# yxtay/transformer-recommenders

Hardware: AMD Instinct MI355X
Metric: user-sequences/sec (train step) MovieLens-1M seq200 d128 @1/2/4/8 GPU (higher is better)
Workload: dtype bf16; 1 GPU; MovieLens-1M-shaped: 3883 items, seq_len=200, d_model=128, 4-layer causal BERT (heads=4, ffn=512), InfoNCELoss over in-batch shared negatives, AdamW; per_gpu_batch=512, global_batch=512, seq_len=200, lengths=dense, loss_heads_evaluated=all 7 + LogitsStatistics (reference training_step), parallelism=dp1, launch=eager launches

## Files before the change

### transformer-recommenders_amd/csrc/common.h

```cpp
#pragma once
#include <hip/hip_runtime.h>
#include <stdint.h>

#include "xfmr_hip.h"

typedef __attribute__((ext_vector_type(8))) __bf16 bf16x8;
typedef __attribute__((ext_vector_type(4))) __bf16 bf16x4;
typedef __attribute__((ext_vector_type(2))) __bf16 bf16x2;
typedef __attribute__((ext_vector_type(16))) float f32x16;

#define XF_WAVE 64

#define XF_LAUNCH_CHECK()                                   \
  do {                                                      \
    if (hipGetLastError() != hipSuccess) return XFMR_EHIP;  \
  } while (0)

static inline bool xf_aligned16(const void* p) { return (reinterpret_cast<uintptr_t>(p) & 15u) == 0; }

__device__ __forceinline__ int xf_lane() { return threadIdx.x & 63; }

__device__ __forceinline__ int xf_acc_row(int r, int lane) { return (r & 3) + 8 * (r >> 2) + 4 * (lane >> 5); }

struct PrecBF16 {
// ... 397 lines not shown
  return fmaf(-p, e, 0.5f);
}
__device__ __forceinline__ float xf_gelu(float x) {
  float e;
  const float ax = fabsf(x);
  return fmaf(ax, xf_phi_minus_half(ax, x, e), 0.5f * x);
}
__device__ __forceinline__ float xf_gelu_both(float x, float& grad) {
  float e;
  const float ax = fabsf(x);
  const float h = xf_phi_minus_half(ax, x, e);
  grad = fmaf(x * 0.3989422804014327f, e, 0.5f + copysignf(h, x));
  return fmaf(ax, h, 0.5f * x);
}
__device__ __forceinline__ float xf_gelu_grad(float x) {
  float e;
  const float h = xf_phi_minus_half(fabsf(x), x, e);
  return fmaf(x * 0.3989422804014327f, e, 0.5f + copysignf(h, x));
}
__device__ __forceinline__ float xf_softplus(float x) {
  return fmaxf(x, 0.f) + 0.6931471805599453f * xf_log2(1.f + xf_exp2(-fabsf(x) * 1.4426950408889634f));
}
__device__ __forceinline__ float xf_sigmoid(float x) {
  const float t = xf_exp2(-fabsf(x) * 1.4426950408889634f);
  return xf_rcp(1.f + t) * (x >= 0.f ? 1.f : t);
}

__device__ __forceinline__ void xf_store_tile_T(float* scratch, const f32x16& acc, float mul, float* base, int64_t stride,
                                             int row0, int row_end) {
  const int lane = xf_lane();
#pragma unroll
  for (int r = 0; r < 16; ++r) scratch[(lane & 31) * 33 + xf_acc_row(r, lane)] = acc[r] * mul;
  __builtin_amdgcn_s_waitcnt(0xc07f);
  __builtin_amdgcn_wave_barrier();
  const int j = lane >> 1, half = lane & 1;
  if (row0 + j < row_end) {
    float* dst = base + (int64_t)(row0 + j) * stride + 16 * half;
#pragma unroll
    for (int u = 0; u < 4; ++u) {
      float4 v;
      v.x = scratch[j * 33 + 16 * half + 4 * u + 0];
      v.y = scratch[j * 33 + 16 * half + 4 * u + 1];
      v.z = scratch[j * 33 + 16 * half + 4 * u + 2];
      v.w = scratch[j * 33 + 16 * half + 4 * u + 3];
      *reinterpret_cast<float4*>(dst + 4 * u) = v;
    }
  }
  __builtin_amdgcn_wave_barrier();
}

__device__ __forceinline__ void xf_store_tile_T(float* scratch, const f32x16& acc, float mul, __bf16* base,
                                                int64_t stride, int row0, int row_end) {
  const int lane = xf_lane();
#pragma unroll
  for (int r = 0; r < 16; ++r) scratch[(lane & 31) * 33 + xf_acc_row(r, lane)] = acc[r] * mul;
  __builtin_amdgcn_s_waitcnt(0xc07f);
  __builtin_amdgcn_wave_barrier();
  const int j = lane >> 1, half = lane & 1;
  if (row0 + j < row_end) {
    __bf16* dst = base + (int64_t)(row0 + j) * stride + 16 * half;
#pragma unroll
    for (int u = 0; u < 2; ++u) {
      bf16x8 v;
#pragma unroll
      for (int e = 0; e < 8; ++e) v[e] = (__bf16)scratch[j * 33 + 16 * half + 8 * u + e];
      *reinterpret_cast<bf16x8*>(dst + 8 * u) = v;
    }
  }
  __builtin_amdgcn_wave_barrier();
}
template <bool S16>
__device__ __forceinline__ void xf_store_tile_T_at(float* scratch, const f32x16& acc, float mul, void* base,
                                                   int64_t off, int64_t stride, int row0, int row_end) {
  if (S16) xf_store_tile_T(scratch, acc, mul, reinterpret_cast<__bf16*>(base) + off, stride, row0, row_end);
  else xf_store_tile_T(scratch, acc, mul, reinterpret_cast<float*>(base) + off, stride, row0, row_end);
}


typedef __attribute__((ext_vector_type(4))) short xf_s16x4;

template <int H>
struct SwzImg {
  static constexpr int CPR = H / 8;
  __device__ static __forceinline__ int swz(int r) {
    if (CPR == 4) return (r >> 2) & 3;
    if (CPR >= 16) return ((r & 3) << 2) | ((r >> 2) & 3);
    return (((r >> 1) & 1) << 2) | ((r & 1) << 1) | ((r >> 2) & 1);
  }
  __device__ static __forceinline__ int off(int r, int c) { return r * H + 8 * (c ^ swz(r)); }

  __device__ static __forceinline__ void tile_nreg(f32x16& acc, const __bf16* A, int arow0, const bf16x8* breg) {
    const int l = xf_lane(), r = arow0 + (l & 31), hh = l >> 5;
#pragma unroll
    for (int s = 0; s < H / 16; ++s) {
      const bf16x8 a = *reinterpret_cast<const bf16x8*>(A + off(r, 2 * s + hh));
      acc = __builtin_amdgcn_mfma_f32_32x32x16_bf16(a, breg[s], acc, 0, 0, 0);
    }
  }
  __device__ static __forceinline__ void tile_nt(f32x16& acc, const __bf16* A, int arow0, const __bf16* B, int brow0) {
    const int l = xf_lane(), ra = arow0 + (l & 31), rb = brow0 + (l & 31), hh = l >> 5;
#pragma unroll
    for (int s = 0; s < H / 16; ++s) {
      const bf16x8 a = *reinterpret_cast<const bf16x8*>(A + off(ra, 2 * s + hh));
      const bf16x8 b = *reinterpret_cast<const bf16x8*>(B + off(rb, 2 * s + hh));
      acc = __builtin_amdgcn_mfma_f32_32x32x16_bf16(a, b, acc, 0, 0, 0);
    }
  }
  __device__ static __forceinline__ void tile_xb_tr(f32x16& acc, const __bf16* img, int hsub, int jrow0,
                                                    const f32x16& x) {
    const int l = xf_lane(), g16 = l >> 4, hh = g16 >> 1, li = l & 15, q = li >> 2, p = li & 3;
    const int col = hsub * 32 + 16 * (g16 & 1) + 4 * p;
    const int c = col >> 3, within = col & 7;
#pragma unroll
    for (int s = 0; s < 2; ++s) {
      bf16x8 b;
#pragma unroll
      for (int j = 0; j < 8; ++j) b[j] = (__bf16)x[8 * s + j];
      union { xf_s16x4 v[2]; bf16x8 f; } a;
#pragma unroll
      for (int t = 0; t < 2; ++t) {
        const int row = jrow0 + 16 * s + 8 * t + 4 * hh + q;
        const __bf16* ptr = img + off(row, c) + within;
        a.v[t] = __builtin_amdgcn_ds_read_tr16_b64_v4i16(
            (__attribute__((address_space(3))) xf_s16x4*)(ptr));
      }
      acc = __builtin_amdgcn_mfma_f32_32x32x16_bf16(a.f, b, acc, 0, 0, 0);
    }
  }
  __device__ static __forceinline__ bf16x8 frag_tr(const __bf16* img, int col0, int k0) {
    const int l = xf_lane(), g16 = l >> 4, li = l & 15, q = li >> 2, p = li & 3;
    const int col = col0 + 16 * (g16 & 1) + 4 * p;
    const int c = col >> 3, within = col & 7;
    union { xf_s16x4 v[2]; bf16x8 f; } a;
#pragma unroll
    for (int t = 0; t < 2; ++t) {
      const int row = k0 + 8 * (g16 >> 1) + 4 * t + q;
      a.v[t] = __builtin_amdgcn_ds_read_tr16_b64_v4i16(
          (__attribute__((address_space(3))) xf_s16x4*)(img + off(row, c) + within));
    }
    return a.f;
  }
  __device__ static __forceinline__ int gather_row(int row0) { return row0 + xf_lane() / CPR; }
  __device__ static __forceinline__ int gather_src_chunk(int row) { return (xf_lane() % CPR) ^ swz(row); }
  static constexpr int kRowsPerInstr = 64 / CPR;
};

__device__ __forceinline__ void xf_glds16(const void* gsrc, void* lds_base) {
  __builtin_amdgcn_global_load_lds((const __attribute__((address_space(1))) void*)gsrc,
                                   (__attribute__((address_space(3))) void*)lds_base, 16, 0, 0);
}
__device__ __forceinline__ void xf_glds16_raw_so(const void* sbase, uint32_t voff, void* lds_base) {
  const unsigned dst = (unsigned)(uintptr_t)(__attribute__((address_space(3))) void*)lds_base;
  unsigned keep;
  asm volatile("s_mov_b32 %0, m0\n\ts_mov_b32 m0, %3\n\ts_nop 0\n\tglobal_load_lds_dwordx4 %1, %2\n\ts_mov_b32 m0, %0"
               : "=&s"(keep)
               : "v"(voff), "s"(sbase), "s"(dst)
               : "memory");
}
template <int N>
__device__ __forceinline__ void xf_wait_vm() {
  __builtin_amdgcn_s_waitcnt((N & 0xF) | ((N >> 4) << 14) | (7 << 4) | (0xF << 8));
}
__device__ __forceinline__ void xf_glds16_raw(const void* gsrc, void* lds_base) {
  const unsigned dst = (unsigned)(uintptr_t)(__attribute__((address_space(3))) void*)lds_base;
  unsigned keep;
  asm volatile("s_mov_b32 %0, m0\n\ts_mov_b32 m0, %2\n\ts_nop 0\n\tglobal_load_lds_dwordx4 %1, off\n\ts_mov_b32 m0, %0"
               : "=&s"(keep)
               : "v"(gsrc), "s"(dst)
               : "memory");
}
```

### transformer-recommenders_amd/csrc/gemm.hip

```cpp
#include <stdio.h>
#include <stdlib.h>

#include <algorithm>
#include <type_traits>

#include "internal.h"

#define XF_PIN_SCALAR(x) asm volatile("" : "+v"(x))
#ifndef XF_LN_DIAG
#define XF_LN_DIAG 0
#endif
#ifndef XF_GEMM_PF
#define XF_GEMM_PF 1
#endif
#ifndef XF_DW_PF
#define XF_DW_PF 1
#endif
#ifdef XF_FFN_STAMP
#define XF_STAMP(i) do { if (stamp_on) st_buf[(i)] = __builtin_readcyclecounter(); } while (0)
#else
#define XF_STAMP(i) do {} while (0)
#endif
#ifndef XF_FFN_ASM_BARRIER
#define XF_FFN_ASM_BARRIER 1
// ... 703 lines not shown
            v[q].x += ax.x; v[q].y += ax.y; v[q].z += ax.z; v[q].w += ax.w;
          } else if (EPI == EPI_GELU_GRAD) {
            if (g.aux_grad) {
              v[q].x *= ax.x; v[q].y *= ax.y; v[q].z *= ax.z; v[q].w *= ax.w;
            } else {
              v[q].x *= xf_gelu_grad(ax.x); v[q].y *= xf_gelu_grad(ax.y);
              v[q].z *= xf_gelu_grad(ax.z); v[q].w *= xf_gelu_grad(ax.w);
            }
          }
        }
        if (EPI == EPI_GELU) st_out(g.C2, o, d);
        st_out(g.C, zoff + o, v);
      }
      __builtin_amdgcn_s_waitcnt(0xc07f);
      __builtin_amdgcn_wave_barrier();
    }
  }
}
template <class P, int BM, int BN, int BK, bool TA, bool TB, int EPI, uint32_t S>
__global__ __launch_bounds__(256, (epi_res_ln(EPI) || EPI == EPI_DX_LNBWD) ? XF_LN_EPI_MIN_WAVES : 1) void gemm_kernel(const GemmArgs g_in) {
  gemm_body<P, BM, BN, BK, TA, TB, EPI, S>(g_in, (int)blockIdx.x);
}
struct GemmGroup { GemmArgs g[4]; int start[5]; };
template <class P, int BM, int BN, int BK, bool TA, bool TB, int EPI, uint32_t S>
__global__ __launch_bounds__(256, 1) void gemm_group_kernel(const GemmGroup p) {
  const int b = (int)blockIdx.x;
  const int i = (b >= p.start[1]) + (b >= p.start[2]) + (b >= p.start[3]);
  gemm_body<P, BM, BN, BK, TA, TB, EPI, S>(p.g[i], b - p.start[i]);
}

struct FfnFwdArgs {
  const __bf16* X;
  const __bf16* W1;
  const float* b1;
  const __bf16* W2;
  __bf16* U;
  __bf16* G;
  int I;
  GemmArgs e;
  unsigned long long* stamps;
};

template <int N, class F>
__device__ __forceinline__ void xf_static_for(F&& fn) {
  if constexpr (N > 0) {
    xf_static_for<N - 1>(fn);
    fn(std::integral_constant<int, N - 1>{});
  }
}
template <int CH>
struct WeightChunk {
  static constexpr int NW = CH / 16, PC = CH / 8, H = 128, LDH = H + 8, LDC = CH + 8;
  bf16x8 reg[NW];
  __device__ __forceinline__ void load_w1(const __bf16* W1, int c, int tid) {
    xf_static_for<NW>([&](auto ic) {
      constexpr int i = decltype(ic)::value;
      const int p = tid + i * 256, row = p >> 4, ch = p & 15;
      reg[i] = *reinterpret_cast<const bf16x8*>(W1 + (int64_t)(c * CH + row) * H + ch * 8);
    });
  }
  __device__ __forceinline__ void commit_w1(__bf16* sW, int tid) const {
    xf_static_for<NW>([&](auto ic) {
      constexpr int i = decltype(ic)::value;
      const int p = tid + i * 256, row = p >> 4, ch = p & 15;
      *reinterpret_cast<bf16x8*>(sW + row * LDH + ch * 8) = reg[i];
    });
  }
  __device__ __forceinline__ void load_w2(const __bf16* W2, int I, int c, int tid) {
    xf_static_for<NW>([&](auto ic) {
      constexpr int i = decltype(ic)::value;
      const int p = tid + i * 256, row = p / PC, ch = p % PC;
      reg[i] = *reinterpret_cast<const bf16x8*>(W2 + (int64_t)row * I + c * CH + ch * 8);
    });
  }
  __device__ __forceinline__ void commit_w2(__bf16* sW, int tid) const {
    xf_static_for<NW>([&](auto ic) {
      constexpr int i = decltype(ic)::value;
      const int p = tid + i * 256, row = p / PC, ch = p % PC;
      *reinterpret_cast<bf16x8*>(sW + row * LDC + ch * 8) = reg[i];
    });
  }
};

template <int CH, bool RE = false>
__global__ __launch_bounds__(256, CH == 128 ? XF_FFN_MIN_WAVES : 3) void ffn_fwd_fused_kernel(const FfnFwdArgs f_in) {
  FfnFwdArgs f = f_in;
  XF_CHAIN_PRIO();
  f.e.drop = xf_drop_resolve(f.e.drop);
  constexpr int H = 128, LDH = H + 8, LDC = CH + 8, BM = 64;
  constexpr int NJ = CH / 64;
  constexpr int W_ELEMS = CH * LDH > H * LDC ? CH * LDH : H * LDC;
  __shared__ __attribute__((aligned(16))) __bf16 sG[BM * LDC];
  __shared__ __attribute__((aligned(16))) __bf16 sW[W_ELEMS];
  __shared__ float sB1[1024];
  static_assert(W_ELEMS >= BM * LDH, "the x tile is staged through sW");
  static_assert(W_ELEMS * 2 >= 4 * 16 * 68 * 4 + 128 * 4, "the LayerNorm epilogue's scratch aliases sW");
  using FR = Frag<PrecBF16, false>;
  const int lane = threadIdx.x & 63, wid = threadIdx.x >> 6, tid = threadIdx.x;
  const int wr = wid >> 1, wc = wid & 1;
  const TileIdx tix = tile_of(1, f.e.nt_m, 1);
  if (!tix.valid) return;
  const int64_t m0 = xf_tile_rows(f.e, tix.m, BM);
  const int64_t M = f.e.M;
  const int I = f.I, nchunk = I / CH;
#ifdef XF_FFN_STAMP
  const bool stamp_on = f.stamps && threadIdx.x == 0;
  unsigned long long* st_buf = f.stamps + (int64_t)blockIdx.x * 64;
#endif
  XF_STAMP(0);

  WeightChunk<CH> wa, wb;
  constexpr int PC = CH / 8;

  {
    uint4 xr[4];
#pragma unroll
    for (int i = 0; i < 4; ++i) {
      const int p = tid + i * 256, row = p >> 4, ch = p & 15;
      xr[i] = make_uint4(0u, 0u, 0u, 0u);
      if (m0 + row < M) xr[i] = *reinterpret_cast<const uint4*>(f.X + (m0 + row) * H + ch * 8);
    }
    wa.load_w1(f.W1, 0, tid);
    wb.load_w2(f.W2, I, 0, tid);
    for (int i = tid; i < I; i += 256) sB1[i] = f.b1[i];
#pragma unroll
    for (int i = 0; i < 4; ++i) {
      const int p = tid + i * 256, row = p >> 4, ch = p & 15;
      *reinterpret_cast<uint4*>(sW + row * LDH + ch * 8) = xr[i];
    }
  }
  __syncthreads();
  bf16x8 xa[H / 16];
#pragma unroll
  for (int ks = 0; ks < H / 16; ++ks) xa[ks] = FR::get(sW, LDH, wr * 32, ks * 16);
  XF_STAMP(1);

  f32x16 accy[2];
#pragma unroll
  for (int j = 0; j < 2; ++j)
#pragma unroll
    for (int r = 0; r < 16; ++r) accy[j][r] = 0.f;

  for (int c = 0; c < nchunk; ++c) {
    XF_LOOP_BARRIER();
    if (c < 2) XF_STAMP(2 + 6 * c);
    wa.commit_w1(sW, tid);
    XF_LOOP_BARRIER();
    if (c < 2) XF_STAMP(3 + 6 * c);
    if (c + 1 < nchunk) wa.load_w1(f.W1, c + 1, tid);
    f32x16 accu[NJ];
#pragma unroll
    for (int j = 0; j < NJ; ++j)
#pragma unroll
      for (int r = 0; r < 16; ++r) accu[j][r] = 0.f;
    {
      bf16x8 fb[2][NJ];
#pragma unroll
      for (int j = 0; j < NJ; ++j) fb[0][j] = FR::get(sW, LDH, wc * (CH / 2) + j * 32, 0);
#pragma unroll
      for (int ks = 0; ks < H / 16; ++ks) {
        if (ks + 1 < H / 16) {
#pragma unroll
          for (int j = 0; j < NJ; ++j) fb[(ks + 1) & 1][j] = FR::get(sW, LDH, wc * (CH / 2) + j * 32, (ks + 1) * 16);
        }
#pragma unroll
        for (int j = 0; j < NJ; ++j) accu[j] = xf_mma(xa[ks], fb[ks & 1][j], accu[j]);
      }
    }
#pragma unroll
    for (int j = 0; j < NJ; ++j) {
      const int col = wc * (CH / 2) + j * 32 + (lane & 31);
      const float b = sB1[c * CH + col];
#pragma unroll
      for (int r = 0; r < 16; ++r) sG[(wr * 32 + xf_acc_row(r, lane)) * LDC + col] = (__bf16)(accu[j][r] + b);
    }
    if (c < 2) XF_STAMP(4 + 6 * c);
    XF_LOOP_BARRIER();
    if (c < 2) XF_STAMP(5 + 6 * c);
#pragma unroll
    for (int i = 0; i < BM * PC / 256; ++i) {
      const int p = tid + i * 256, row = p / PC, ch = p % PC;
      float4* cell = reinterpret_cast<float4*>(sG + row * LDC + ch * 8);
      const float4 u8 = *cell;
      const float4 g8 = xf_gelu_bf16x8(u8);
      if (m0 + row < M) {
        if (f.U) *reinterpret_cast<float4*>(f.U + (m0 + row) * I + c * CH + ch * 8) = u8;
        if (f.G) *reinterpret_cast<float4*>(f.G + (m0 + row) * I + c * CH + ch * 8) = g8;
      }
      *cell = g8;
    }
    wb.commit_w2(sW, tid);
    if (c < 2) XF_STAMP(6 + 6 * c);
    XF_LOOP_BARRIER();
    if (c < 2) XF_STAMP(7 + 6 * c);
    if (c + 1 < nchunk) wb.load_w2(f.W2, I, c + 1, tid);
#pragma unroll
    for (int ks = 0; ks < CH / 16; ++ks) {
      const bf16x8 fa = FR::get(sG, LDC, wr * 32, ks * 16);
      bf16x8 fb[2];
#pragma unroll
      for (int j = 0; j < 2; ++j) fb[j] = FR::get(sW, LDC, wc * 64 + j * 32, ks * 16);
#pragma unroll
      for (int j = 0; j < 2; ++j) accy[j] = xf_mma(fa, fb[j], accy[j]);
    }
  }
  XF_STAMP(14);
  __syncthreads();
  XF_STAMP(15);
  epi_drop_res_ln_64x128<RE ? 1 : 0>(accy, reinterpret_cast<unsigned char*>(sW), f.e, m0, wid, lane);
  XF_STAMP(16);
}

struct FfnBwdArgs {
  const __bf16* DY;
  const __bf16* W2;
  const __bf16* U;
  const __bf16* W1;
  __bf16* DI;
  int I;
  GemmArgs e;
};

template <bool RING>
__global__ __launch_bounds__(256, 3) void ffn_bwd_dx_fused_kernel(const FfnBwdArgs f_in) {
  FfnBwdArgs f = f_in;
  XF_CHAIN_PRIO();
  f.e.drop = xf_drop_resolve(f.e.drop); f.e.drop2 = xf_drop_resolve(f.e.drop2);
  constexpr int H = 128, BM = 64, CH = 64, LDH = H + 8, LDC = CH + 8;
  constexpr int LDF = CH + 4;
  constexpr int EPI_BYTES = (4 * 16 * 68 + 2 * 2 * 2 * 16 * 2 + 2 * 3 * 128) * 4;
  using FN = Frag<PrecBF16, false>;
  using FT = Frag<PrecBF16, true>;
  const int lane = threadIdx.x & 63, wid = threadIdx.x >> 6, tid = threadIdx.x;
  const int wr = wid >> 1, wc = wid & 1;
  const TileIdx tix = tile_of(1, f.e.nt_m, 1);
  if (!tix.valid) return;
  const int64_t m0 = xf_tile_rows(f.e, tix.m, BM);
  const int64_t M = f.e.M;
  const int I = f.I, nchunk = I / CH;

  bf16x8 ur[2];
  auto load_u = [&](int c) {
    xf_static_for<2>([&](auto ic) {
      constexpr int i = decltype(ic)::value;
      const int p = tid + i * 256, row = p >> 3, ch = p & 7;
      bf16x8 z;
#pragma unroll
      for (int e = 0; e < 8; ++e) z[e] = (__bf16)0.f;
      if (m0 + row < M) z = *reinterpret_cast<const bf16x8*>(f.U + (m0 + row) * I + c * CH + ch * 8);
      ur[i] = z;
    });
  };
  auto di_piece = [&](const float* sF, const int i) {
    const int p = tid + i * 256, row = p >> 3, ch = p & 7;
    const float4 g0 = *reinterpret_cast<const float4*>(sF + row * LDF + ch * 8);
    const float4 g1 = *reinterpret_cast<const float4*>(sF + row * LDF + ch * 8 + 4);
    const bf16x8 u8 = ur[i];
    bf16x8 d8;
    d8[0] = (__bf16)(g0.x * xf_gelu_grad((float)u8[0])); d8[1] = (__bf16)(g0.y * xf_gelu_grad((float)u8[1]));
    d8[2] = (__bf16)(g0.z * xf_gelu_grad((float)u8[2])); d8[3] = (__bf16)(g0.w * xf_gelu_grad((float)u8[3]));
    d8[4] = (__bf16)(g1.x * xf_gelu_grad((float)u8[4])); d8[5] = (__bf16)(g1.y * xf_gelu_grad((float)u8[5]));
    d8[6] = (__bf16)(g1.z * xf_gelu_grad((float)u8[6])); d8[7] = (__bf16)(g1.w * xf_gelu_grad((float)u8[7]));
    return d8;
  };
  auto store_dg = [&](float* sF, const f32x16& accg) {
    const int col = wc * 32 + (lane & 31);
#pragma unroll
    for (int r = 0; r < 16; ++r) sF[(wr * 32 + xf_acc_row(r, lane)) * LDF + col] = accg[r];
  };

  f32x16 accx[2];
#pragma unroll
  for (int j = 0; j < 2; ++j)
#pragma unroll
    for (int r = 0; r < 16; ++r) accx[j][r] = 0.f;

  if constexpr (RING) {
    constexpr int F_BYTES = BM * LDF * 4, G_BYTES = BM * LDC * 2, W2_BYTES = H * CH * 2, W1_BYTES = CH * H * 2;
    __shared__ __attribute__((aligned(16))) unsigned char smem[F_BYTES + G_BYTES + W1_BYTES];
    static_assert(W2_BYTES <= F_BYTES, "the W2 chunk image lands in sF's bytes");
    static_assert(BM * LDH * 2 <= G_BYTES + W1_BYTES, "the dy tile is staged over sG and the W1 image");
    static_assert(EPI_BYTES <= F_BYTES + G_BYTES, "the epilogue's scratch aliases sF and sG");
    static_assert(F_BYTES % 1024 == 0 && G_BYTES % 1024 == 0, "DMA targets on 1-KiB instruction boundaries");
    float* const sF = reinterpret_cast<float*>(smem);
    __bf16* const sW2 = reinterpret_cast<__bf16*>(smem);
    __bf16* const sG = reinterpret_cast<__bf16*>(smem + F_BYTES);
    __bf16* const sW1 = reinterpret_cast<__bf16*>(smem + F_BYTES + G_BYTES);
    __bf16* const sY = sG;
    using I2 = SwzImg<CH>;
    using I1 = SwzImg<H>;
    const int w = __builtin_amdgcn_readfirstlane(wid);
    auto issue_w2 = [&](int c) {
      xf_static_for<4>([&](auto jc) {
// ... 366 lines not shown
  }();
  int64_t want = (1024 + tiles - 1) / tiles;
  if (want > max_split) want = max_split;
  if (want < 1) want = 1;
  int64_t chunk = (M + want - 1) / want;
  chunk = ((chunk + 127) / 128) * 128;
  if (M >= 4096 && chunk < 256) chunk = 256;
  if (chunk < 64) chunk = 64;
  *k_chunk = (int)chunk;
  return (int)((M + chunk - 1) / chunk);
}
int dw_split_bound(int64_t M, int N, int K) {
  int k_chunk;
  const int64_t tiles = ((N + 63) / 64) * ((K + 63) / 64);
  int64_t want = (1024 + tiles - 1) / tiles;
  if (want > 256) want = 256;
  const int64_t by_rows = (M + 127) / 128;
  const int64_t bound = by_rows < want ? by_rows : want;
  const int plan = dw_split_plan(M, N, K, &k_chunk);
  return bound > plan ? (int)bound : plan;
}

int set_ln_residual(GemmArgs& g, const float* residual, const XfLnResidual* res, XfSeed seed) {
  if ((residual != nullptr) == (res != nullptr)) return XFMR_EINVAL;
  g.R = residual;
  if (!res) return xf_aligned16(residual) ? XFMR_OK : XFMR_EALIGN;
  if (!res->pre || !res->mean || !res->rstd || !res->gamma || !res->beta) return XFMR_EINVAL;
  if (!xf_aligned16(res->pre) || !xf_aligned16(res->gamma) || !xf_aligned16(res->beta)) return XFMR_EALIGN;
  g.rp_pre = res->pre; g.rp_mean = res->mean; g.rp_rstd = res->rstd; g.rp_gamma = res->gamma; g.rp_beta = res->beta;
  g.rp_drop = xf_make_dropout(res->dropout_p, seed, res->site);
  return XFMR_OK;
}

int linear_ln_fwd(const void* x, const float* w, const float* bias, float* pre, int64_t M, int32_t N, int32_t K,
                  const float* residual, const XfLnResidual* res, float dropout_p, XfSeed seed, uint32_t site,
                  const float* gamma, const float* beta, float eps, float* y, void* y16, float* mean, float* rstd,
                  int32_t precision, uint32_t s16, hipStream_t st) {
  if (!x || !w || !pre || !gamma || !beta || (!y && !y16) || !mean || !rstd || M <= 0 || K <= 0) return XFMR_EINVAL;
  if (N != 128 || (K & 7)) return XFMR_EUNSUPPORTED;
  if (precision != XFMR_PREC_BF16) return XFMR_EUNSUPPORTED;
  if (!xf_aligned16(x) || !xf_aligned16(w) || !xf_aligned16(pre) || (y && !xf_aligned16(y))) return XFMR_EALIGN;
  GemmArgs g{};
  g.A = x; g.B = w; g.C = pre; g.lda = K; g.ldb = K; g.ldc = N; g.M = M; g.N = N; g.K = K; g.k_chunk = 0;
  g.bias = bias; g.s16 = s16 & (XF_S16_A | XF_S16_B);
  if (const int rc = set_ln_residual(g, residual, res, seed)) return rc;
  g.drop = xf_make_dropout(dropout_p, seed, site);
  g.ln_gamma = gamma; g.ln_beta = beta; g.ln_eps = eps; g.Y = y; g.Y16 = y16; g.ln_mean = mean; g.ln_rstd = rstd;
  if (!res) return dispatch_gemm<false, false, EPI_DROP_RES_LN, XF_S16_A, (XF_S16_A | XF_S16_B)>(g, 1, precision, st);
  if (g.s16 != (XF_S16_A | XF_S16_B)) return XFMR_EUNSUPPORTED;
  if (g.rp_drop.on) return launch_gemm<PrecBF16, false, false, EPI_DROP_RES_LN_RED, (XF_S16_A | XF_S16_B)>(g, 1, st);
  return launch_gemm<PrecBF16, false, false, EPI_DROP_RES_LN_RE, (XF_S16_A | XF_S16_B)>(g, 1, st);
}

int ffn_fwd_fused(const void* x16, const void* w1_16, const float* b1, const void* w2_16, const float* b2, void* u16,
                  void* g16, float* pre, int64_t M, int32_t H, int32_t I, const float* residual, const XfLnResidual* res,
                  float dropout_p, XfSeed seed, uint32_t site, const float* gamma, const float* beta, float eps, float* y,
                  void* y16, float* mean, float* rstd, hipStream_t st) {
  if (!x16 || !w1_16 || !b1 || !w2_16 || !pre || !gamma || !beta || (!y && !y16) || !mean || !rstd || M <= 0)
    return XFMR_EINVAL;
  if (H != 128 || I <= 0 || (I % 128) || I > 1024) return XFMR_EUNSUPPORTED;
  if (res && res->dropout_p > 0.f) return XFMR_EUNSUPPORTED;
  if (!xf_aligned16(x16) || !xf_aligned16(w1_16) || !xf_aligned16(w2_16) || !xf_aligned16(pre) ||
      (y && !xf_aligned16(y)) || (u16 && !xf_aligned16(u16)) || (g16 && !xf_aligned16(g16)) || (y16 && !xf_aligned16(y16)) || !xf_aligned16(b1) ||
      (b2 && !xf_aligned16(b2)) || !xf_aligned16(gamma) || !xf_aligned16(beta))
    return XFMR_EALIGN;
  FfnFwdArgs f{};
  f.X = (const __bf16*)x16; f.W1 = (const __bf16*)w1_16; f.b1 = b1; f.W2 = (const __bf16*)w2_16; f.U = (__bf16*)u16; f.G = (__bf16*)g16;
  f.I = I;
#ifdef XF_FFN_STAMP
  if (const char* e = getenv("XFMR_FFN_STAMPS")) f.stamps = (unsigned long long*)strtoull(e, nullptr, 0);
#endif
  GemmArgs& g = f.e;
  g.C = pre; g.ldc = H; g.M = M; g.N = H; g.K = I; g.bias = b2;
  if (const int rc = set_ln_residual(g, residual, res, seed)) return rc;
  g.drop = xf_make_dropout(dropout_p, seed, site);
  g.ln_gamma = gamma; g.ln_beta = beta; g.ln_eps = eps; g.Y = y; g.Y16 = y16; g.ln_mean = mean; g.ln_rstd = rstd;
  g.nt_n = 1; g.nt_z = 1;
  xf_plan_row_tiles(g, 64);
  const int64_t groups = (g.nt_m + 7) / 8;
  if (groups * 8 > 0x7fffffffll) return XFMR_EUNSUPPORTED;
  const char* ce = getenv("XFMR_FFN_CHUNK");
  const int chunk = ce ? atoi(ce) : 64;
  const dim3 grid((unsigned)(groups * 8));
  if (chunk == 64 && res) hipLaunchKernelGGL((ffn_fwd_fused_kernel<64, true>), grid, dim3(256), 0, st, f);
  else if (chunk == 64) hipLaunchKernelGGL((ffn_fwd_fused_kernel<64, false>), grid, dim3(256), 0, st, f);
  else if (res) hipLaunchKernelGGL((ffn_fwd_fused_kernel<128, true>), grid, dim3(256), 0, st, f);
  else hipLaunchKernelGGL((ffn_fwd_fused_kernel<128, false>), grid, dim3(256), 0, st, f);
  XF_LAUNCH_CHECK();
  return XFMR_OK;
}

}


extern "C" {

int xf_dw_split_plan(int64_t M, int32_t N, int32_t K, int* k_chunk) { return dw_split_plan(M, N, K, k_chunk); }

int xf_rowsum(float* dst, const float* src, int64_t rows, int64_t cols, hipStream_t st) {
  return launch_rowsum(dst, src, rows, cols, rows, st);
}

int xf_ln_row_tiles(int64_t M) {
  GemmArgs g{};
  g.M = M;
  xf_plan_row_tiles(g, 64);
  return g.nt_m;
}

int xf_linear_fwd_ex(const void* x, const float* w, const float* bias, void* y, int64_t M, int32_t N, int32_t K,
                     int32_t epilogue, const float* residual, void* aux_out, float dropout_p, XfSeed seed,
                     uint32_t site, int32_t precision, uint32_t s16, hipStream_t st) {
  if (!x || !w || !y || M <= 0 || N <= 0 || K <= 0) return XFMR_EINVAL;
  if ((K & 3) || (N & 3)) return XFMR_EUNSUPPORTED;
  if (!xf_aligned16(x) || !xf_aligned16(w) || !xf_aligned16(y)) return XFMR_EALIGN;
  if ((s16 & ~XF_AUX_GELU_GRAD) && precision != XFMR_PREC_BF16) return XFMR_EINVAL;
  if ((s16 & (XF_S16_A | XF_S16_B | XF_S16_C | XF_S16_P)) && ((K & 7) || (N & 7))) return XFMR_EUNSUPPORTED;
  GemmArgs g{};
  g.A = x; g.B = w; g.C = y; g.lda = K; g.ldb = K; g.ldc = N; g.M = M; g.N = N; g.K = K; g.k_chunk = 0;
  g.bias = bias; g.R = residual; g.C2 = aux_out; g.P = nullptr; g.s16 = s16 & (XF_S16_A | XF_S16_B | XF_S16_C);
  g.aux_grad = (s16 & XF_AUX_GELU_GRAD) != 0;
  g.drop = xf_make_dropout(dropout_p, seed, site);
  switch (epilogue) {
    case XFMR_EPI_BIAS:
      g.R = nullptr;
      return dispatch_gemm<false, false, EPI_STORE, XF_S16_C, (XF_S16_C | XF_S16_B),
                           (XF_S16_A | XF_S16_B | XF_S16_C)>(g, 1, precision, st);
    case XFMR_EPI_BIAS_GELU:
      if (!aux_out) return XFMR_EINVAL;
      return dispatch_gemm<false, false, EPI_GELU, XF_S16_C, (XF_S16_C | XF_S16_B),
                           (XF_S16_A | XF_S16_B | XF_S16_C)>(g, 1, precision, st);
    case XFMR_EPI_BIAS_DROP_RES:
      if (!residual) return XFMR_EINVAL;
      return dispatch_gemm<false, false, EPI_DROP_RES, XF_S16_A, (XF_S16_A | XF_S16_B)>(g, 1, precision, st);
    default:
      return XFMR_EINVAL;
  }
}

int xf_linear_ln_fwd_ex(const void* x, const float* w, const float* bias, float* pre, int64_t M, int32_t N, int32_t K,
                        const float* residual, float dropout_p, XfSeed seed, uint32_t site, const float* gamma,
                        const float* beta, float eps, float* y, void* y16, float* mean, float* rstd, int32_t precision,
                        uint32_t s16, hipStream_t st) {
  if (!residual || !y) return XFMR_EINVAL;
  return linear_ln_fwd(x, w, bias, pre, M, N, K, residual, nullptr, dropout_p, seed, site, gamma, beta, eps, y, y16, mean,
                       rstd, precision, s16, st);
}
int xf_linear_ln_fwd_re(const void* x, const float* w, const float* bias, float* pre, int64_t M, int32_t N, int32_t K,
                        const XfLnResidual* res, float dropout_p, XfSeed seed, uint32_t site, const float* gamma,
                        const float* beta, float eps, float* y, void* y16, float* mean, float* rstd, int32_t precision,
                        uint32_t s16, hipStream_t st) {
  if (!res) return XFMR_EINVAL;
  return linear_ln_fwd(x, w, bias, pre, M, N, K, nullptr, res, dropout_p, seed, site, gamma, beta, eps, y, y16, mean, rstd,
                       precision, s16, st);
}

int xfmr_linear_fwd(const float* x, const float* w, const float* bias, float* y, int64_t M, int32_t N, int32_t K,
                    int32_t epilogue, const float* residual, float* aux_out, float dropout_p, uint64_t seed,
                    uint32_t site, int32_t precision, void* stream) {
  return xf_linear_fwd_ex(x, w, bias, y, M, N, K, epilogue, residual, aux_out, dropout_p, seed, site, precision, 0,
                          (hipStream_t)stream);
}

int xf_ffn_fwd_fused_ex(const void* x16, const void* w1_16, const float* b1, const void* w2_16, const float* b2,
                        void* u16, void* g16, float* pre, int64_t M, int32_t H, int32_t I, const float* residual, float dropout_p,
                        XfSeed seed, uint32_t site, const float* gamma, const float* beta, float eps, float* y,
                        void* y16, float* mean, float* rstd, hipStream_t st) {
// ... 254 lines not shown
```

Baseline: 164,800 sequences/s.

## Stream FFN forward weight chunks into swizzled LDS via direct global-to-LDS DMA

Adds a RING variant of the fused FFN forward kernel for 64-column chunks. W1 and W2 chunks are loaded with global_load_lds straight into XOR-swizzled LDS images instead of being staged through registers and committed with explicit LDS stores. The next W1 chunk is issued during the current chunk's GELU phase, and waits are done with vmcnt counters. Compile-time static_asserts check the gather/read mapping, and the new path is the default, with an environment flag to fall back. This frees VGPRs and removes the register-to-LDS store instructions, at the cost of more intricate waitcnt ordering and a larger combined LDS footprint.

```diff
diff --git a/transformer-recommenders_amd/csrc/common.h b/transformer-recommenders_amd/csrc/common.h
--- a/transformer-recommenders_amd/csrc/common.h
+++ b/transformer-recommenders_amd/csrc/common.h
@@ -503,12 +503,12 @@
 template <int H>
 struct SwzImg {
   static constexpr int CPR = H / 8;
-  __device__ static __forceinline__ int swz(int r) {
+  __host__ __device__ static __forceinline__ constexpr int swz(int r) {
     if (CPR == 4) return (r >> 2) & 3;
     if (CPR >= 16) return ((r & 3) << 2) | ((r >> 2) & 3);
     return (((r >> 1) & 1) << 2) | ((r & 1) << 1) | ((r >> 2) & 1);
   }
-  __device__ static __forceinline__ int off(int r, int c) { return r * H + 8 * (c ^ swz(r)); }
+  __host__ __device__ static __forceinline__ constexpr int off(int r, int c) { return r * H + 8 * (c ^ swz(r)); }
 
   __device__ static __forceinline__ void tile_nreg(f32x16& acc, const __bf16* A, int arow0, const bf16x8* breg) {
     const int l = xf_lane(), r = arow0 + (l & 31), hh = l >> 5;
@@ -561,8 +561,10 @@
     }
     return a.f;
   }
-  __device__ static __forceinline__ int gather_row(int row0) { return row0 + xf_lane() / CPR; }
-  __device__ static __forceinline__ int gather_src_chunk(int row) { return (xf_lane() % CPR) ^ swz(row); }
+  __host__ __device__ static __forceinline__ constexpr int gather_row_of(int row0, int lane) { return row0 + lane / CPR; }
+  __host__ __device__ static __forceinline__ constexpr int gather_src_chunk_of(int row, int lane) { return (lane % CPR) ^ swz(row); }
+  __device__ static __forceinline__ int gather_row(int row0) { return gather_row_of(row0, xf_lane()); }
+  __device__ static __forceinline__ int gather_src_chunk(int row) { return gather_src_chunk_of(row, xf_lane()); }
   static constexpr int kRowsPerInstr = 64 / CPR;
 };
 
diff --git a/transformer-recommenders_amd/csrc/gemm.hip b/transformer-recommenders_amd/csrc/gemm.hip
--- a/transformer-recommenders_amd/csrc/gemm.hip
+++ b/transformer-recommenders_amd/csrc/gemm.hip
@@ -809,7 +809,58 @@
   }
 };
 
-template <int CH, bool RE = false>
+struct FfnFwdRingMaps {
+  static constexpr int H = 128, CH = 64;
+  using I1 = SwzImg<H>;
+  using I2 = SwzImg<H>;
+  static constexpr int w1_row0(int w, int j) { return 16 * w + I1::kRowsPerInstr * j; }
+  static constexpr int w2_row0(int w, int j) { return 16 * w + I2::kRowsPerInstr * j; }
+  static constexpr int w1_src(int c, int i, int q) { return (c * CH + i) * H + 8 * q; }
+  static constexpr int w2_src(int I, int c, int i, int q) { return (2 * i + (q >> 3)) * I + c * CH + 8 * (q & 7); }
+  template <class IMG>
+  static constexpr int dma_lds_byte(int row0, int lane) { return row0 * IMG::CPR * 16 + lane * 16; }
+  static constexpr int w1_read(int n, int k) { return I1::off(n, k >> 3); }
+  static constexpr int w2_read(int n, int k) { return I2::off(n >> 1, 8 * (n & 1) + (k >> 3)); }
+  __device__ static __forceinline__ bf16x8 w1_frag(const __bf16* img, int n0, int k0) {
+    const int l = xf_lane();
+    return *reinterpret_cast<const bf16x8*>(img + w1_read(n0 + (l & 31), k0 + 8 * (l >> 5)));
+  }
+  __device__ static __forceinline__ bf16x8 w2_frag(const __bf16* img, int n0, int k0) {
+    const int l = xf_lane();
+    return *reinterpret_cast<const bf16x8*>(img + w2_read(n0 + (l & 31), k0 + 8 * (l >> 5)));
+  }
+  template <bool IS_W1>
+  static constexpr bool image_ok(int I, int c) {
+    using IMG = std::conditional_t<IS_W1, I1, I2>;
+    constexpr int ROWS = 64, SLOTS = ROWS * IMG::CPR;
+    int src[SLOTS] = {}, hits[SLOTS] = {};
+    for (int w = 0; w < 4; ++w)
+      for (int j = 0; j < 4; ++j)
+        for (int lane = 0; lane < 64; ++lane) {
+          const int row0 = IS_W1 ? w1_row0(w, j) : w2_row0(w, j);
+          const int n = IMG::gather_row_of(row0, lane), q = IMG::gather_src_chunk_of(n, lane);
+          const int b = dma_lds_byte<IMG>(row0, lane);
+          if (n < 0 || n >= ROWS || q < 0 || q >= IMG::CPR || b < 0 || (b & 15) || b / 16 >= SLOTS) return false;
+          ++hits[b / 16];
+          src[b / 16] = IS_W1 ? w1_src(c, n, q) : w2_src(I, c, n, q);
+        }
+    for (int s = 0; s < SLOTS; ++s)
+      if (hits[s] != 1) return false;
+    for (int n = 0; n < (IS_W1 ? CH : H); ++n)
+      for (int k = 0; k < (IS_W1 ? H : CH); k += 8) {
+        const int b = 2 * (IS_W1 ? w1_read(n, k) : w2_read(n, k));
+        if (b < 0 || (b & 15) || b / 16 >= SLOTS) return false;
+        if (src[b / 16] != (IS_W1 ? (c * CH + n) * H + k : n * I + c * CH + k)) return false;
+      }
+    return true;
+  }
+};
+static_assert(FfnFwdRingMaps::image_ok<true>(512, 0) && FfnFwdRingMaps::image_ok<true>(1024, 15),
+              "W1 chunk image: the gather covers every slot once and the swizzled read finds W1[c 64 + n][k]");
+static_assert(FfnFwdRingMaps::image_ok<false>(512, 0) && FfnFwdRingMaps::image_ok<false>(1024, 15),
+              "W2 chunk image: the gather covers every slot once and the swizzled read finds W2[n][c 64 + k]");
+
+template <int CH, bool RE = false, bool RING = false>
 __global__ __launch_bounds__(256, CH == 128 ? XF_FFN_MIN_WAVES : 3) void ffn_fwd_fused_kernel(const FfnFwdArgs f_in) {
   FfnFwdArgs f = f_in;
   XF_CHAIN_PRIO();
@@ -817,11 +868,6 @@
   constexpr int H = 128, LDH = H + 8, LDC = CH + 8, BM = 64;
   constexpr int NJ = CH / 64;
   constexpr int W_ELEMS = CH * LDH > H * LDC ? CH * LDH : H * LDC;
-  __shared__ __attribute__((aligned(16))) __bf16 sG[BM * LDC];
-  __shared__ __attribute__((aligned(16))) __bf16 sW[W_ELEMS];
-  __shared__ float sB1[1024];
-  static_assert(W_ELEMS >= BM * LDH, "the x tile is staged through sW");
-  static_assert(W_ELEMS * 2 >= 4 * 16 * 68 * 4 + 128 * 4, "the LayerNorm epilogue's scratch aliases sW");
   using FR = Frag<PrecBF16, false>;
   const int lane = threadIdx.x & 63, wid = threadIdx.x >> 6, tid = threadIdx.x;
   const int wr = wid >> 1, wc = wid & 1;
@@ -835,107 +881,244 @@
   unsigned long long* st_buf = f.stamps + (int64_t)blockIdx.x * 64;
 #endif
   XF_STAMP(0);
-
-  WeightChunk<CH> wa, wb;
-  constexpr int PC = CH / 8;
-
-  {
-    uint4 xr[4];
-#pragma unroll
-    for (int i = 0; i < 4; ++i) {
-      const int p = tid + i * 256, row = p >> 4, ch = p & 15;
-      xr[i] = make_uint4(0u, 0u, 0u, 0u);
-      if (m0 + row < M) xr[i] = *reinterpret_cast<const uint4*>(f.X + (m0 + row) * H + ch * 8);
-    }
-    wa.load_w1(f.W1, 0, tid);
-    wb.load_w2(f.W2, I, 0, tid);
-    for (int i = tid; i < I; i += 256) sB1[i] = f.b1[i];
-#pragma unroll
-    for (int i = 0; i < 4; ++i) {
-      const int p = tid + i * 256, row = p >> 4, ch = p & 15;
-      *reinterpret_cast<uint4*>(sW + row * LDH + ch * 8) = xr[i];
-    }
-  }
-  __syncthreads();
-  bf16x8 xa[H / 16];
-#pragma unroll
-  for (int ks = 0; ks < H / 16; ++ks) xa[ks] = FR::get(sW, LDH, wr * 32, ks * 16);
-  XF_STAMP(1);
-
-  f32x16 accy[2];
-#pragma unroll
-  for (int j = 0; j < 2; ++j)
-#pragma unroll
-    for (int r = 0; r < 16; ++r) accy[j][r] = 0.f;
-
-  for (int c = 0; c < nchunk; ++c) {
+  if constexpr (RING) {
+    static_assert(CH == 64, "the LDS-DMA form exists for 64-column chunks");
+    using I1 = FfnFwdRingMaps::I1;
+    using I2 = FfnFwdRingMaps::I2;
+    constexpr int W1_BYTES = CH * H * 2, W2_BYTES = H * CH * 2, G_BYTES = BM * LDC * 2, B1_BYTES = 1024 * 4;
+    constexpr int X_BYTES = BM * LDH * 2;
+    constexpr int EPI_BYTES = 4 * 16 * 68 * 4 + 128 * 4;
+    __shared__ __attribute__((aligned(1024))) unsigned char smem[W1_BYTES + W2_BYTES + G_BYTES + B1_BYTES];
+    static_assert(W1_BYTES % 1024 == 0 && W2_BYTES % 1024 == 0 && G_BYTES % 1024 == 0, "every region starts on a 1-KiB boundary");
+    static_assert(X_BYTES <= W2_BYTES + G_BYTES, "the x tile is staged over the W2 image and the head of sG");
+    static_assert(EPI_BYTES <= W1_BYTES + W2_BYTES, "the LayerNorm epilogue's scratch aliases the two images");
+    static_assert(sizeof(smem) <= 46080, "three workgroups per CU");
+    __bf16* const sW1 = reinterpret_cast<__bf16*>(smem);
+    __bf16* const sW2 = reinterpret_cast<__bf16*>(smem + W1_BYTES);
+    __bf16* const sG = reinterpret_cast<__bf16*>(smem + W1_BYTES + W2_BYTES);
+    float* const sB1 = reinterpret_cast<float*>(smem + W1_BYTES + W2_BYTES + G_BYTES);
+    __bf16* const sX = sW2;
+    const int w = __builtin_amdgcn_readfirstlane(wid);
+    auto issue_w1 = [&](int c) {
+      xf_static_for<4>([&](auto jc) {
+        constexpr int j = decltype(jc)::value;
+        const int row0 = FfnFwdRingMaps::w1_row0(w, j), i = I1::gather_row(row0);
+        xf_glds16_raw_so(f.W1, (uint32_t)FfnFwdRingMaps::w1_src(c, i, I1::gather_src_chunk(i)) * 2u,
+                         smem + FfnFwdRingMaps::dma_lds_byte<I1>(row0, 0));
+      });
+    };
+    auto issue_w2 = [&](int c) {
+      xf_static_for<4>([&](auto jc) {
+        constexpr int j = decltype(jc)::value;
+        const int row0 = FfnFwdRingMaps::w2_row0(w, j), i = I2::gather_row(row0);
+        xf_glds16_raw_so(f.W2, (uint32_t)FfnFwdRingMaps::w2_src(I, c, i, I2::gather_src_chunk(i)) * 2u,
+                         smem + W1_BYTES + FfnFwdRingMaps::dma_lds_byte<I2>(row0, 0));
+      });
+    };
+
+    issue_w1(0);
+    {
+      uint4 xr[4];
+#pragma unroll
+      for (int i = 0; i < 4; ++i) {
+        const int p = tid + i * 256, row = p >> 4, ch = p & 15;
+        xr[i] = make_uint4(0u, 0u, 0u, 0u);
+        if (m0 + row < M) xr[i] = *reinterpret_cast<const uint4*>(f.X + (m0 + row) * H + ch * 8);
+      }
+      for (int i = tid; i < I; i += 256) sB1[i] = f.b1[i];
+#pragma unroll
+      for (int i = 0; i < 4; ++i) {
+        const int p = tid + i * 256, row = p >> 4, ch = p & 15;
+        *reinterpret_cast<uint4*>(sX + row * LDH + ch * 8) = xr[i];
+      }
+    }
     XF_LOOP_BARRIER();
-    if (c < 2) XF_STAMP(2 + 6 * c);
-    wa.commit_w1(sW, tid);
-    XF_LOOP_BARRIER();
-    if (c < 2) XF_STAMP(3 + 6 * c);
-    if (c + 1 < nchunk) wa.load_w1(f.W1, c + 1, tid);
-    f32x16 accu[NJ];
-#pragma unroll
-    for (int j = 0; j < NJ; ++j)
-#pragma unroll
-      for (int r = 0; r < 16; ++r) accu[j][r] = 0.f;
+    bf16x8 xa[H / 16];
+#pragma unroll
+    for (int ks = 0; ks < H / 16; ++ks) xa[ks] = FR::get(sX, LDH, wr * 32, ks * 16);
+    XF_STAMP(1);
+
+    f32x16 accy[2];
+#pragma unroll
+    for (int j = 0; j < 2; ++j)
+#pragma unroll
+      for (int r = 0; r < 16; ++r) accy[j][r] = 0.f;
+
+    for (int c = 0; c < nchunk; ++c) {
+      if (c < 2) XF_STAMP(2 + 6 * c);
+      xf_wait_vm<0>();
+      XF_LOOP_BARRIER();
+      if (c < 2) XF_STAMP(3 + 6 * c);
+      issue_w2(c);
+      f32x16 accu;
+#pragma unroll
+      for (int r = 0; r < 16; ++r) accu[r] = 0.f;
+      {
+        bf16x8 fb[2];
+        fb[0] = FfnFwdRingMaps::w1_frag(sW1, wc * 32, 0);
+#pragma unroll
+        for (int ks = 0; ks < H / 16; ++ks) {
+          if (ks + 1 < H / 16) fb[(ks + 1) & 1] = FfnFwdRingMaps::w1_frag(sW1, wc * 32, (ks + 1) * 16);
+          accu = xf_mma(xa[ks], fb[ks & 1], accu);
+        }
+      }
+      {
+        const int col = wc * 32 + (lane & 31);
+        const float b = sB1[c * CH + col];
+#pragma unroll
+        for (int r = 0; r < 16; ++r) sG[(wr * 32 + xf_acc_row(r, lane)) * LDC + col] = (__bf16)(accu[r] + b);
+      }
+      if (c < 2) XF_STAMP(4 + 6 * c);
+      XF_LOOP_BARRIER();
+      if (c < 2) XF_STAMP(5 + 6 * c);
+      if (c + 1 < nchunk) issue_w1(c + 1);
+      float4 u8[2], g8[2];
+      xf_static_for<2>([&](auto ic) {
+        constexpr int i = decltype(ic)::value;
+        const int p = tid + i * 256, row = p >> 3, ch = p & 7;
+        u8[i] = *reinterpret_cast<const float4*>(sG + row * LDC + ch * 8);
+        g8[i] = xf_gelu_bf16x8(u8[i]);
+      });
+#pragma unroll
+      for (int i = 0; i < 2; ++i) asm volatile("" : "+v"(g8[i].x), "+v"(g8[i].y), "+v"(g8[i].z), "+v"(g8[i].w));
+      if (c + 1 < nchunk) xf_wait_vm<4>();
+      else xf_wait_vm<0>();
+      asm volatile("" ::: "memory");
+      xf_static_for<2>([&](auto ic) {
+        constexpr int i = decltype(ic)::value;
+        const int p = tid + i * 256, row = p >> 3, ch = p & 7;
+        if (m0 + row < M) {
+          if (f.U) *reinterpret_cast<float4*>(f.U + (m0 + row) * I + c * CH + ch * 8) = u8[i];
+          if (f.G) *reinterpret_cast<float4*>(f.G + (m0 + row) * I + c * CH + ch * 8) = g8[i];
+        }
+        *reinterpret_cast<float4*>(sG + row * LDC + ch * 8) = g8[i];
+      });
+      if (c < 2) XF_STAMP(6 + 6 * c);
+      XF_LOOP_BARRIER();
+      if (c < 2) XF_STAMP(7 + 6 * c);
+#pragma unroll
+      for (int ks = 0; ks < CH / 16; ++ks) {
+        const bf16x8 fa = FR::get(sG, LDC, wr * 32, ks * 16);
+        bf16x8 fb[2];
+#pragma unroll
+        for (int j = 0; j < 2; ++j) fb[j] = FfnFwdRingMaps::w2_frag(sW2, wc * 64 + j * 32, ks * 16);
+#pragma unroll
+        for (int j = 0; j < 2; ++j) accy[j] = xf_mma(fa, fb[j], accy[j]);
+      }
+    }
+    XF_STAMP(14);
+    __syncthreads();
+    XF_STAMP(15);
+    epi_drop_res_ln_64x128<RE ? 1 : 0>(accy, smem, f.e, m0, wid, lane);
+    XF_STAMP(16);
+  } else {
+    __shared__ __attribute__((aligned(16))) __bf16 sG[BM * LDC];
+    __shared__ __attribute__((aligned(16))) __bf16 sW[W_ELEMS];
+    __shared__ float sB1[1024];
+    static_assert(W_ELEMS >= BM * LDH, "the x tile is staged through sW");
+    static_assert(W_ELEMS * 2 >= 4 * 16 * 68 * 4 + 128 * 4, "the LayerNorm epilogue's scratch aliases sW");
+
+    WeightChunk<CH> wa, wb;
+    constexpr int PC = CH / 8;
+
     {
-      bf16x8 fb[2][NJ];
-#pragma unroll
-      for (int j = 0; j < NJ; ++j) fb[0][j] = FR::get(sW, LDH, wc * (CH / 2) + j * 32, 0);
-#pragma unroll
-      for (int ks = 0; ks < H / 16; ++ks) {
-        if (ks + 1 < H / 16) {
-#pragma unroll
-          for (int j = 0; j < NJ; ++j) fb[(ks + 1) & 1][j] = FR::get(sW, LDH, wc * (CH / 2) + j * 32, (ks + 1) * 16);
+      uint4 xr[4];
+#pragma unroll
+      for (int i = 0; i < 4; ++i) {
+        const int p = tid + i * 256, row = p >> 4, ch = p & 15;
+        xr[i] = make_uint4(0u, 0u, 0u, 0u);
+        if (m0 + row < M) xr[i] = *reinterpret_cast<const uint4*>(f.X + (m0 + row) * H + ch * 8);
+      }
+      wa.load_w1(f.W1, 0, tid);
+      wb.load_w2(f.W2, I, 0, tid);
+      for (int i = tid; i < I; i += 256) sB1[i] = f.b1[i];
+#pragma unroll
+      for (int i = 0; i < 4; ++i) {
+        const int p = tid + i * 256, row = p >> 4, ch = p & 15;
+        *reinterpret_cast<uint4*>(sW + row * LDH + ch * 8) = xr[i];
+      }
+    }
+    __syncthreads();
+    bf16x8 xa[H / 16];
+#pragma unroll
+    for (int ks = 0; ks < H / 16; ++ks) xa[ks] = FR::get(sW, LDH, wr * 32, ks * 16);
+    XF_STAMP(1);
+
+    f32x16 accy[2];
+#pragma unroll
+    for (int j = 0; j < 2; ++j)
+#pragma unroll
+      for (int r = 0; r < 16; ++r) accy[j][r] = 0.f;
+
+    for (int c = 0; c < nchunk; ++c) {
+      XF_LOOP_BARRIER();
+      if (c < 2) XF_STAMP(2 + 6 * c);
+      wa.commit_w1(sW, tid);
+      XF_LOOP_BARRIER();
+      if (c < 2) XF_STAMP(3 + 6 * c);
+      if (c + 1 < nchunk) wa.load_w1(f.W1, c + 1, tid);
+      f32x16 accu[NJ];
+#pragma unroll
+      for (int j = 0; j < NJ; ++j)
+#pragma unroll
+        for (int r = 0; r < 16; ++r) accu[j][r] = 0.f;
+      {
+        bf16x8 fb[2][NJ];
+#pragma unroll
+        for (int j = 0; j < NJ; ++j) fb[0][j] = FR::get(sW, LDH, wc * (CH / 2) + j * 32, 0);
+#pragma unroll
+        for (int ks = 0; ks < H / 16; ++ks) {
+          if (ks + 1 < H / 16) {
+#pragma unroll
+            for (int j = 0; j < NJ; ++j) fb[(ks + 1) & 1][j] = FR::get(sW, LDH, wc * (CH / 2) + j * 32, (ks + 1) * 16);
+          }
+#pragma unroll
+          for (int j = 0; j < NJ; ++j) accu[j] = xf_mma(xa[ks], fb[ks & 1][j], accu[j]);
         }
-#pragma unroll
-        for (int j = 0; j < NJ; ++j) accu[j] = xf_mma(xa[ks], fb[ks & 1][j], accu[j]);
-      }
-    }
-#pragma unroll
-    for (int j = 0; j < NJ; ++j) {
-      const int col = wc * (CH / 2) + j * 32 + (lane & 31);
-      const float b = sB1[c * CH + col];
-#pragma unroll
-      for (int r = 0; r < 16; ++r) sG[(wr * 32 + xf_acc_row(r, lane)) * LDC + col] = (__bf16)(accu[j][r] + b);
-    }
-    if (c < 2) XF_STAMP(4 + 6 * c);
-    XF_LOOP_BARRIER();
-    if (c < 2) XF_STAMP(5 + 6 * c);
-#pragma unroll
-    for (int i = 0; i < BM * PC / 256; ++i) {
-      const int p = tid + i * 256, row = p / PC, ch = p % PC;
-      float4* cell = reinterpret_cast<float4*>(sG + row * LDC + ch * 8);
-      const float4 u8 = *cell;
-      const float4 g8 = xf_gelu_bf16x8(u8);
-      if (m0 + row < M) {
-        if (f.U) *reinterpret_cast<float4*>(f.U + (m0 + row) * I + c * CH + ch * 8) = u8;
-        if (f.G) *reinterpret_cast<float4*>(f.G + (m0 + row) * I + c * CH + ch * 8) = g8;
-      }
-      *cell = g8;
-    }
-    wb.commit_w2(sW, tid);
-    if (c < 2) XF_STAMP(6 + 6 * c);
-    XF_LOOP_BARRIER();
-    if (c < 2) XF_STAMP(7 + 6 * c);
-    if (c + 1 < nchunk) wb.load_w2(f.W2, I, c + 1, tid);
-#pragma unroll
-    for (int ks = 0; ks < CH / 16; ++ks) {
-      const bf16x8 fa = FR::get(sG, LDC, wr * 32, ks * 16);
-      bf16x8 fb[2];
-#pragma unroll
-      for (int j = 0; j < 2; ++j) fb[j] = FR::get(sW, LDC, wc * 64 + j * 32, ks * 16);
-#pragma unroll
-      for (int j = 0; j < 2; ++j) accy[j] = xf_mma(fa, fb[j], accy[j]);
-    }
-  }
-  XF_STAMP(14);
-  __syncthreads();
-  XF_STAMP(15);
-  epi_drop_res_ln_64x128<RE ? 1 : 0>(accy, reinterpret_cast<unsigned char*>(sW), f.e, m0, wid, lane);
-  XF_STAMP(16);
+      }
+#pragma unroll
+      for (int j = 0; j < NJ; ++j) {
+        const int col = wc * (CH / 2) + j * 32 + (lane & 31);
+        const float b = sB1[c * CH + col];
+#pragma unroll
+        for (int r = 0; r < 16; ++r) sG[(wr * 32 + xf_acc_row(r, lane)) * LDC + col] = (__bf16)(accu[j][r] + b);
+      }
+      if (c < 2) XF_STAMP(4 + 6 * c);
+      XF_LOOP_BARRIER();
+      if (c < 2) XF_STAMP(5 + 6 * c);
+#pragma unroll
+      for (int i = 0; i < BM * PC / 256; ++i) {
+        const int p = tid + i * 256, row = p / PC, ch = p % PC;
+        float4* cell = reinterpret_cast<float4*>(sG + row * LDC + ch * 8);
+        const float4 u8 = *cell;
+        const float4 g8 = xf_gelu_bf16x8(u8);
+        if (m0 + row < M) {
+          if (f.U) *reinterpret_cast<float4*>(f.U + (m0 + row) * I + c * CH + ch * 8) = u8;
+          if (f.G) *reinterpret_cast<float4*>(f.G + (m0 + row) * I + c * CH + ch * 8) = g8;
+        }
+        *cell = g8;
+      }
+      wb.commit_w2(sW, tid);
+      if (c < 2) XF_STAMP(6 + 6 * c);
+      XF_LOOP_BARRIER();
+      if (c < 2) XF_STAMP(7 + 6 * c);
+      if (c + 1 < nchunk) wb.load_w2(f.W2, I, c + 1, tid);
+#pragma unroll
+      for (int ks = 0; ks < CH / 16; ++ks) {
+        const bf16x8 fa = FR::get(sG, LDC, wr * 32, ks * 16);
+        bf16x8 fb[2];
+#pragma unroll
+        for (int j = 0; j < 2; ++j) fb[j] = FR::get(sW, LDC, wc * 64 + j * 32, ks * 16);
+#pragma unroll
+        for (int j = 0; j < 2; ++j) accy[j] = xf_mma(fa, fb[j], accy[j]);
+      }
+    }
+    XF_STAMP(14);
+    __syncthreads();
+    XF_STAMP(15);
+    epi_drop_res_ln_64x128<RE ? 1 : 0>(accy, reinterpret_cast<unsigned char*>(sW), f.e, m0, wid, lane);
+    XF_STAMP(16);
+  }
 }
 
 struct FfnBwdArgs {
@@ -1468,7 +1651,11 @@
   const char* ce = getenv("XFMR_FFN_CHUNK");
   const int chunk = ce ? atoi(ce) : 64;
   const dim3 grid((unsigned)(groups * 8));
-  if (chunk == 64 && res) hipLaunchKernelGGL((ffn_fwd_fused_kernel<64, true>), grid, dim3(256), 0, st, f);
+  auto env_on = [](const char* name) { const char* e = getenv(name); return e && *e && *e != '0'; };
+  const bool ring = !env_on("XFMR_FFN_FWD_REG_STAGE") && !env_on("XFMR_FFN_REG_STAGE");
+  if (chunk == 64 && ring && res) hipLaunchKernelGGL((ffn_fwd_fused_kernel<64, true, true>), grid, dim3(256), 0, st, f);
+  else if (chunk == 64 && ring) hipLaunchKernelGGL((ffn_fwd_fused_kernel<64, false, true>), grid, dim3(256), 0, st, f);
+  else if (chunk == 64 && res) hipLaunchKernelGGL((ffn_fwd_fused_kernel<64, true>), grid, dim3(256), 0, st, f);
   else if (chunk == 64) hipLaunchKernelGGL((ffn_fwd_fused_kernel<64, false>), grid, dim3(256), 0, st, f);
   else if (res) hipLaunchKernelGGL((ffn_fwd_fused_kernel<128, true>), grid, dim3(256), 0, st, f);
   else hipLaunchKernelGGL((ffn_fwd_fused_kernel<128, false>), grid, dim3(256), 0, st, f);
```

Result: no change. 166,100 sequences/s (median of 6 runs) (+0.8%).
